# automl/learning_environments

Hardware: AMD Instinct MI355X
Metric: NES worker-evaluations/sec (full inner-loop train+eval) at pop=64 per GPU (higher is better)
Workload: dtype f32

## Files before the change

learning_environments_amd/csrc/dueling_se_inner_loop.hip:

```cpp
#include "lenv_gemm.cuh"
#include "lenv_ln.cuh"
#include "lenv_icm.cuh"
#include "lenv_wavechain_host.h"

namespace lenv {

constexpr int D_MAXL = 3;
constexpr int D_MAXW = 128;
constexpr int D_MAXH = 512;
constexpr int D_MAXB = 640;
constexpr int D_MAXI = 128;

struct DuelArena { int64_t a_online, a_target, a_m, a_v, a_grad, a_xs, a_xs2, a_act[D_MAXL], a_feat, a_v1, a_a1, a_t[6], a_dbuf[5], a_xh[D_MAXL], a_rstd, end; };
constexpr DuelArena duel_arena(int S, int H, int F, int L, int B, int T, int64_t P, bool ln = false)
{
    DuelArena a{};
    int64_t off = 0;
#define LENV_TAKE64(n) ([&]() { int64_t r_ = off; off += ((int64_t)(n) + 3) & ~(int64_t)3; return r_; }())
    a.a_online = LENV_TAKE64(P); a.a_target = LENV_TAKE64(P); a.a_m = LENV_TAKE64(P); a.a_v = LENV_TAKE64(P); a.a_grad = LENV_TAKE64(P);
    const int64_t rows = B > T ? B : T;
    const int W = H > F ? H : F;
    a.a_xs = LENV_TAKE64(rows * S); a.a_xs2 = LENV_TAKE64(rows * S);
    for (int l = 0; l < D_MAXL; ++l) a.a_act[l] = LENV_TAKE64(l < L ? (int64_t)B * H : 0);
    a.a_feat = LENV_TAKE64((int64_t)B * F); a.a_v1 = LENV_TAKE64((int64_t)B * F); a.a_a1 = LENV_TAKE64((int64_t)B * F);
// ... 218 lines not shown
            n_act = (int)rec[4]; learn_it = (int)rec[5]; n_test_ep = (int)rec[6]; train_steps = (int)rec[7]; test_steps = (int)rec[8];
            episodes_run = (int)rec[9];
            eps_g = __longlong_as_double(rec[11]); b1pow = __longlong_as_double(rec[12]); b2pow = __longlong_as_double(rec[13]);
            icm_pows[0] = __longlong_as_double(rec[14]); icm_pows[1] = __longlong_as_double(rec[15]);
        }
    }

    auto obs_of = [&](const double *st, float *obs) { real_env_obs(env_id, st, obs); };

    GemmQueue gq(cmds);
    constexpr int LNBUF = GemmShape<D_MAXI>::PS_FLOATS + GemmShape<D_MAXI>::QS_FLOATS;
    auto queue_forward = [&](const float *par, const float *X, int I, float *const *hid, float *featb, float *v1b, float *a1b, int slot,
                             float *const *xhs = nullptr, float *rstds = nullptr) {
        const float *in = X;
        int n_in = S;
        for (int l = 0; l < L; ++l) {
            if (ln && l >= 1) {
                gq.gemm(in, n_in, 1, par + po.oWf[l], n_in, 1, I, H, n_in, epi_bias(hid[l], H, 0, par + po.obf[l]));
                gq.run<D_MAXI>(Ps, Qs);
                ln_rows_forward<LNBUF>(Ps, hid[l], I, H, par + po.oLN, par + po.oLN + H, xhs ? xhs[l] : nullptr, rstds ? rstds + (int64_t)l * CFG_B : nullptr, act_id, prelu);
            } else gq.gemm(in, n_in, 1, par + po.oWf[l], n_in, 1, I, H, n_in, epi_bias_act(hid[l], H, par + po.obf[l], act_id, prelu));
            in = hid[l]; n_in = H;
        }
        if (plain) {
            gq.gemm(in, n_in, 1, par + po.oWf[L], n_in, 1, I, A, n_in, epi_bias(Advb + slot * RBH * A, A, 0, par + po.obf[L]));
            return;
        }
        gq.gemm(in, n_in, 1, par + po.oWf[L], n_in, 1, I, F, n_in, epi_bias(featb, F, 0, par + po.obf[L]));
        gq.gemm(featb, F, 1, par + po.oWv1, F, 1, I, F, F, epi_bias_act(v1b, F, par + po.obv1, act_id, prelu));
        gq.gemm(featb, F, 1, par + po.oWa1, F, 1, I, F, F, epi_bias_act(a1b, F, par + po.oba1, act_id, prelu));
        gq.gemm(v1b, F, 1, par + po.oWv2, F, 1, I, 1, F, epi_bias(Vb + slot * RBH, 1, 0, par + po.obv2));
        gq.gemm(a1b, F, 1, par + po.oWa2, F, 1, I, A, F, epi_bias(Advb + slot * RBH * A, A, 0, par + po.oba2));
    };
    auto finish_q = [&](int slot, int I, float *q_out, bool global_mean) {
        if (plain) {
            const float *src = Advb + slot * RBH * A;
            for (int e = tid; e < I * A; e += DNT) q_out[e] = src[e];
            __syncthreads();
            return;
        }
        const float *Vs = Vb + slot * RBH, *As = Advb + slot * RBH * A;
        if (global_mean) {
            if (tid == 0) {
                float sum = 0.0f;
                for (int e = 0; e < I * A; ++e) sum = sum + As[e];
                ctrl[8] = sum / (float)(I * A);
            }
            __syncthreads();
            const float mean = ctrl[8];
            for (int e = tid; e < I * A; e += DNT) q_out[e] = Vs[e / A] + (As[e] - mean);
        } else {
            for (int i = tid; i < I; i += DNT) {
                float sum = 0.0f;
                for (int aa = 0; aa < A; ++aa) sum = sum + As[i * A + aa];
                const float mean = sum / (float)A;
                for (int aa = 0; aa < A; ++aa) q_out[i * A + aa] = Vs[i] + (As[i * A + aa] - mean);
            }
        }
        __syncthreads();
    };
    auto forward = [&](const float *par, const float *X, int I, float *const *hid, float *featb, float *v1b, float *a1b,
                       float *q_out, bool global_mean) {
        queue_forward(par, X, I, hid, featb, v1b, a1b, 0);
        gq.run<D_MAXI>(Ps, Qs);
        finish_q(0, I, q_out, global_mean);
    };

    auto icm_step = [&]() {
        if constexpr (ICM) {
            IcmStep st{ gq, Ps, Qs, arena, a.a_icm, ctrl, 12, icm, icm_pows, cfg.icm_lr, cfg.icm_beta, cfg.icm_eta, cfg.adam_beta1, cfg.adam_beta2,
                        cfg.adam_eps, B, xs, S, xs2, S, false };
            const int Ai = icm.Ai;
            icm_train_and_reward<D_MAXI>(st, [&](int b, int i) { return Ai == 1 ? dAdv[b * A] : ((int)dAdv[b * A] == i ? 1.0f : 0.0f); },
                                         [&](int b, float r) { dAdv[b * A + 1] = dAdv[b * A + 1] + r; });
        }
    };

    float *hid_s[D_MAXL], *hid_t[D_MAXL];
    for (int l = 0; l < D_MAXL; ++l) { hid_s[l] = arena + AV(a_act[l]); hid_t[l] = arena + AV(a_t[l]); }
    float *xh_s[D_MAXL], *rstd_s = arena + AV(a_rstd);
    for (int l = 0; l < D_MAXL; ++l) xh_s[l] = arena + AV(a_xh[l]);
    float *feat_t = arena + AV(a_t[3]), *v1_t = arena + AV(a_t[4]), *a1_t = arena + AV(a_t[5]);

    auto test_phase = [&]() {
        if (tid < T) {
            double st[4];
            const int64_t row = (int64_t)n_test_ep + tid;
            if (tape) {
                if (row >= a.tapes.test_reset_stride) { status = -5; for (int i = 0; i < 4; ++i) st[i] = 0.0; }
                else for (int i = 0; i < 4; ++i) st[i] = a.tapes.test_reset[(chain * a.tapes.test_reset_stride + row) * 4 + i];
            } else {
                real_env_reset_draw(env_id, key, STREAM_TEST_RESET, row, st);
            }
            for (int i = 0; i < 4; ++i) dstate[tid * 4 + i] = st[i];
            ep_rew[tid] = 0.0f; alive[tid] = 1; tlen[tid] = 0;
        }
        if (tid == 0) ictrl[0] = 0;
        __syncthreads();
        float *xt = xs2;
        for (int t = 0; t < cfg.max_steps; t += k_rep) {
            if (tid < T) { float obs[8]; obs_of(dstate + tid * 4, obs); for (int i = 0; i < S; ++i) xt[tid * S + i] = obs[i]; }
            __syncthreads();
            forward(online, xt, T, hid_t, feat_t, v1_t, a1_t, qv, false);
            if (tid < T && alive[tid]) {
                int am = 0; float best = qv[tid * A];
                for (int aa = 1; aa < A; ++aa) { const float v = qv[tid * A + aa]; if (v > best) { best = v; am = aa; } }
                double st[4] = { dstate[tid * 4], dstate[tid * 4 + 1], dstate[tid * 4 + 2], dstate[tid * 4 + 3] };
                double rsum = 0.0;
                int nstep = 0;
                for (int r_ = 0; r_ < k_rep; ++r_) {
                    double rew; int dn;
                    real_env_step(env_id, st, am, rew, dn);
                    rsum = rsum + rew;
                    ++nstep;
                    if (tlen[tid] + nstep >= cfg.max_steps) dn = 1;
                    if (dn) { alive[tid] = 0; break; }
                }
                for (int i = 0; i < 4; ++i) dstate[tid * 4 + i] = st[i];
                ep_rew[tid] = ep_rew[tid] + (float)rsum;
                tlen[tid] = tlen[tid] + nstep;
                atomicAdd(const_cast<int *>(&ictrl[0]), nstep);
            }
            __syncthreads();
            int any = 0;
            for (int e = 0; e < T; ++e) any |= alive[e];
            if (!any) break;
        }
        if (tid < T) ret[tid] = (double)ep_rew[tid];
        n_test_ep += T;
        __syncthreads();
        test_steps += ictrl[0];
        __syncthreads();
    };

    const bool budgeted = cfg.step_budget > 0;
    const bool no_test_env = FIXED ? false : cfg.test_mode == 1;
// ... 12 lines not shown
                else for (int i = 0; i < 4; ++i) st0[i] = a.tapes.train_reset[(chain * a.tapes.train_reset_stride + episode) * 4 + i];
            } else {
                real_env_reset_draw(env_id, key, STREAM_TRAIN_RESET, episode, st0);
            }
            float obs[8];
            obs_of(st0, obs);
            for (int i = 0; i < S; ++i) state[i] = obs[i];
            if (reward_env) { for (int i = 0; i < 4; ++i) tstate[i] = st0[i]; ictrl[5] = 0; }
        }
        __syncthreads();
        int ep_len = 0, env_steps = 0;
        float tr_reward = 0.0f;
        for (int t = 0; t < cfg.max_steps; t += k_rep) {
            PT_MARK(9);
            const int size_after = train_steps + 1 < rb_cap ? train_steps + 1 : rb_cap;
            const int new_pos = train_steps % rb_cap;
            if (tid == 0) {
                double u;
                if (tape) { if (train_steps >= a.tapes.eps_uniform_stride) { status = -2; u = 1.0; } else u = a.tapes.eps_uniform[chain * a.tapes.eps_uniform_stride + train_steps]; }
                else u = u64_to_unit(rng_u64(key, STREAM_EPS, (uint64_t)train_steps));
                int explored = u < eps_g, action = -1;
                if (explored) {
                    if (tape) { if (n_act >= a.tapes.rand_action_stride) { status = -3; action = 0; } else action = a.tapes.rand_action[chain * a.tapes.rand_action_stride + n_act]; }
                    else action = (int)u64_to_below(rng_u64(key, STREAM_ACTION, (uint64_t)n_act), (uint32_t)A);
                }
                ictrl[1] = explored; ictrl[2] = action;
            }
            __syncthreads();
            const int explored = ictrl[1];
            if (explored) ++n_act;
            if (!explored) {
                for (int i = tid; i < S; i += DNT) xs2[i] = state[i];
                __syncthreads();
                forward(online, xs2, 1, hid_t, feat_t, v1_t, a1_t, qv, false);
                if (tid == 0) {
                    int am = 0; float best = qv[0];
                    for (int aa = 1; aa < A; ++aa) if (qv[aa] > best) { best = qv[aa]; am = aa; }
                    ictrl[2] = am;
                }
                __syncthreads();
            }
            const int action = ictrl[2];
            PT_MARK(0);
            if (reward_env) {
                auto rn_phi = [&](const float *obs, int slot) {
                    const float *rnp = seL > 1 ? arena + a.a_se_mid : rn_w;
                    const float *W0 = rnp, *b0 = rnp + Hse * Drn;
                    for (int j = tid; j < Hse; j += DNT) {
                        float z = 0.0f;
                        for (int k = 0; k < Drn; ++k) z = fma32(obs[k], W0[j * Drn + k], z);
                        rn_h[j] = act_fwd(se_act_id, cfg.se_prelu, z + b0[j]);
                    }
                    __syncthreads();
                    const float *hp = rn_h, *Wl = b0 + Hse;
                    float *hn = se_h2;
                    for (int l = 1; l < seL; ++l) {
                        const float *bl = Wl + Hse * Hse;
                        for (int j = tid; j < Hse; j += DNT) {
                            float z = 0.0f;
                            for (int k = 0; k < Hse; ++k) z = fma32(hp[k], Wl[j * Hse + k], z);
                            z = z + bl[j];
                            hn[j] = se_ln ? z : act_fwd(se_act_id, cfg.se_prelu, z);
                        }
                        __syncthreads();
                        if (se_ln) {
                            if (tid == 0) {
                                float sm = 0.0f, sv = 0.0f;
// ... 127 lines not shown
                a.out.trace_action[k] = action | (explored << 16);
                for (int i = 0; i < S; ++i) { a.out.trace_state[k * S + i] = newrow[i]; a.out.trace_next_state[k * S + i] = newrow[S + 1 + i]; }
                a.out.trace_reward_done[k * 2] = newrow[2 * S + 1]; a.out.trace_reward_done[k * 2 + 1] = newrow[2 * S + 2];
            }
            const float done_now = newrow[2 * S + 2];
            tr_reward = tr_reward + newrow[2 * S + 1];
            __syncthreads();
            if (tid < S) state[tid] = newrow[S + 1 + tid];
            ep_len += k_rep; ++train_steps;
            __syncthreads();
            PT_MARK(1);

            if (learning) {
                for (int b = tid; b < B; b += DNT) {
                    const int64_t n = (int64_t)learn_it * B + b;
                    int idx;
                    if (tape) {
                        if (n >= a.tapes.replay_idx_stride) { status = -4; idx = 0; } else idx = a.tapes.replay_idx[chain * a.tapes.replay_idx_stride + n];
                        if (idx < 0 || idx >= size_after) { status = -6; idx = 0; }
                    } else idx = (int)rng_replay_below(key, (uint64_t)n, (uint32_t)size_after);
                    const float *row = rb + (int64_t)idx * RS;
                    for (int i = 0; i < S; ++i) { xs[b * S + i] = row[i]; xs2[b * S + i] = row[S + 1 + i]; }
                    dAdv[b * A + 0] = row[S];
                    dAdv[b * A + 1] = row[2 * S + 1];
                    dq[b] = row[2 * S + 2];
                }
                __syncthreads();
                icm_step();
                PT_MARK(2);
                queue_forward(online, xs2, B, hid_t, feat_t, v1_t, a1_t, 1);
                queue_forward(target, xs2, B, hid_t, feat_t, v1_t, a1_t, 2);
                queue_forward(online, xs, B, hid_s, feat_s, v1_s, a1_s, 0, xh_s, rstd_s);
                gq.run<D_MAXI>(Ps, Qs);
                finish_q(1, B, qv + B * A, true);
                finish_q(2, B, qv + 2 * B * A, true);
                finish_q(0, B, qv, true);
                PT_MARK(3);
                for (int b = tid; b < B; b += DNT) {
                    const float g32 = (float)cfg.gamma, norm = (float)(2.0 / (double)B);
                    const int ab = (int)dAdv[b * A + 0];
                    const float r = dAdv[b * A + 1], d = dq[b];
                    int am = 0; float best = qv[(B + b) * A];
                    for (int aa = 1; aa < A; ++aa) { const float v = qv[(B + b) * A + aa]; if (v > best) { best = v; am = aa; } }
                    const float t1 = g32 * qv[(2 * B + b) * A + am];
                    const float t2 = 1.0f - d;
                    const float y = r + t1 * t2;
                    dq[b] = norm * (qv[b * A + ab] - y);
                    Vb[b] = (float)ab;
                }
                __syncthreads();
                if (tid == 0) {
                    float s_dq = 0.0f;
                    for (int b = 0; b < B; ++b) s_dq = s_dq + dq[b];
                    ctrl[9] = plain ? 0.0f : (-s_dq) / (float)(B * A);
                    b1pow *= cfg.adam_beta1; b2pow *= cfg.adam_beta2;
                    ctrl[10] = (float)(-(lr / (1.0 - b1pow)));
                    ctrl[11] = (float)__builtin_sqrt(1.0 - b2pow);
                }
                __syncthreads();
                {
                    const float mean_grad = ctrl[9];
                    for (int e = tid; e < B * A; e += DNT) {
                        const int b = e / A, aa = e - b * A;
                        const float g = aa == (int)Vb[b] ? dq[b] : 0.0f;
                        dAdv[e] = plain ? g : g + mean_grad;
                    }
                }
                __syncthreads();
                PT_MARK(4);
// ... 433 lines not shown
```

learning_environments_amd/csrc/dueling_wavechain.hip:

```cpp
#include "lenv_wavechain.cuh"
#ifndef WCT_NO_FUSED_OPT
#define WCT_FUSED_OPT
#endif
#include "lenv_wavechain_host.h"

namespace lenv {

using namespace wc;

struct WcShape { int env, S, A, Hse, T, q_act, se_act, kind; };
constexpr WcShape kWcShapes[] = {
    { -1, 2, 2, 1, 1, 0, 0, 1 },
    { LENV_ENV_ACROBOT, 6, 3, 128, 10, LENV_ACT_RELU, LENV_ACT_LEAKYRELU, 1 },
    { LENV_ENV_ACROBOT, 6, 3, 128, 10, LENV_ACT_RELU, LENV_ACT_LEAKYRELU, 0 },
};
constexpr int WC_B = 128, WC_H = 128;

namespace wcp {
constexpr int oW1t = 0, ob1 = 8 * W, oW2t = ob1 + W, ob2 = oW2t + IMG, oW3t = ob2 + W, ob3 = oW3t + IMG, oWv1t = ob3 + W, obv1 = oWv1t + IMG,
              oWa1t = obv1 + W, oba1 = oWa1t + IMG, oWh = oba1 + W, obh = oWh + 4 * W, PW = obh + 4;
static_assert(PW % 4 == 0, "float4 passes");
}

enum { D_H1 = 0, D_H2, D_FEAT, D_V1, D_A1, S_F1, S_DFEAT, S_DH2, S_DH1,
// ... 660 lines not shown
        sm_bias[i] = par[off + j];
    }
    for (int i = tid; i < 4 * W + 4; i += NT) sm_wh[i] = par[oWh + i];
    StageRegs sr;
    WSUB_DECL;
    stage_load_direct(par + oW2t, L, sr);
    stage_store_direct(bufA, L, sr);
    __syncthreads();
    WSUB_MARK(48);
    float r16[2][16], rf[2][64];
    f32x16 acc;
    auto xch = [&](int job) { return bufB + (quad * 2 + job) * 4096; };
#pragma unroll
    for (int j = 0; j < 2; ++j) {
        if (j < nj) {
            const float *X = pass == 0 ? xs2 : (j == 0 ? xs : xs2);
#pragma unroll
            for (int v = 0; v < 16; ++v) acc[v] = 0.0f;
            const lfloat *w1 = sm_w1t + L.h * W + 32 * jt + L.li;
#pragma unroll
            for (int t = 0; t < S / 2; ++t) acc = __builtin_amdgcn_mfma_f32_32x32x2f32(w1[2 * t * W], X[row * S + 2 * t + L.h], acc, 0, 0, 0);
#pragma unroll
            for (int g4 = 0; g4 < 4; ++g4) {
                const f32x4 bv = *(const lf4 *)(sm_bias + 32 * jt + 8 * g4 + 4 * L.h);
#pragma unroll
                for (int cc = 0; cc < 4; ++cc) r16[j][4 * g4 + cc] = act_fwd(ACT, prelu, acc[4 * g4 + cc] + bv[cc]);
            }
            if (pass == 1 && j == 0) piece_store(dump_of(D_H1, blk), jt, L.lane, r16[j]);
            tile16_to_operand(r16[j]);
            xch_put(xch(j), jt, L.lane, r16[j]);
        }
    }
    barrier_lds();
#pragma unroll
    for (int j = 0; j < 2; ++j) if (j < nj) xch_get(xch(j), L.lane, rf[j]);
    barrier_lds();
    WSUB_MARK(49);
#pragma unroll 1
    for (int l = 0; l < NL; ++l) {
#pragma unroll
        for (int j = 0; j < 2; ++j) {
            if (j < nj) {
#pragma unroll
                for (int v = 0; v < 16; ++v) acc[v] = 0.0f;
                chain_tile(bufA, jt, L, rf[j], acc);
                const lfloat *bb = sm_bias + (l + 1) * W + 32 * jt + 4 * L.h;
#pragma unroll
                for (int g4 = 0; g4 < 4; ++g4) {
                    const f32x4 bv = *(const lf4 *)(bb + 8 * g4);
#pragma unroll
                    for (int cc = 0; cc < 4; ++cc) {
                        const float z = acc[4 * g4 + cc] + bv[cc];
                        r16[j][4 * g4 + cc] = l == 1 ? z : act_fwd(ACT, prelu, z);
                    }
                }
                if (pass == 1 && j == 0) {
                    piece_store(dump_of(l == 0 ? D_H2 : (l == 1 ? D_FEAT : (l == 2 ? D_V1 : D_A1)), blk), jt, L.lane, r16[j]);
                    if (l >= 2 || PL) {
                        gfloat *rm = (gfloat *)dump_of(l == 2 ? R_V1 : R_A1, 0) + row * W + 32 * jt + 4 * L.h;
#pragma unroll
                        for (int g4 = 0; g4 < 4; ++g4) *(gf4 *)(rm + 8 * g4) = f32x4{r16[j][4 * g4], r16[j][4 * g4 + 1], r16[j][4 * g4 + 2], r16[j][4 * g4 + 3]};
                    }
                }
                tile16_to_operand(r16[j]);
            }
        }
        WSUB_MARK(50);
        if (!PL && l < 2) {
#pragma unroll
            for (int j = 0; j < 2; ++j) if (j < nj) xch_put(xch(j), jt, L.lane, r16[j]);
            barrier_lds();
#pragma unroll
            for (int j = 0; j < 2; ++j) if (j < nj) xch_get(xch(j), L.lane, rf[j]);
            stage_load_direct(par + (l == 0 ? oW3t : oWv1t), L, sr);
            stage_store_direct(bufA, L, sr);
            barrier_lds();
        } else if (!PL && l == 2) {
#pragma unroll
            for (int j = 0; j < 2; ++j) if (j < nj) xch_put(xch(j), jt, L.lane, r16[j]);
            barrier_lds();
            stage_load_direct(par + oWa1t, L, sr);
            stage_store_direct(bufA, L, sr);
            barrier_lds();
        } else {
            barrier_lds();
#pragma unroll
            for (int j = 0; j < 2; ++j) if (j < nj) xch_put(bufA + (quad * 2 + j) * 4096, jt, L.lane, r16[j]);
            barrier_lds();
            const int hd = wave & 1, tj = nj == 2 ? (wave >> 1) & 1 : 0, tq = nj == 2 ? wave >> 2 : wave >> 1;
            if ((nj == 2 || wave < 4) && !(PL && hd == 0)) {
                float rh[64];
                xch_get((hd == 0 ? bufB : bufA) + (tq * 2 + tj) * 4096, L.lane, rh);
                f32x16 hacc;
#pragma unroll
                for (int v = 0; v < 16; ++v) hacc[v] = 0.0f;
                const int col = hd == 0 ? 0 : 1 + (L.li < A ? L.li : A - 1);
                const lfloat *wh = sm_wh + L.h * 4 + col;
#pragma unroll
                for (int t = 0; t < 64; ++t) hacc = __builtin_amdgcn_mfma_f32_32x32x2f32(wh[2 * t * 4], rh[breg_of(t)], hacc, 0, 0, 0);
                if (L.h == 0) {
                    const int slot = pass == 0 ? 2 : tj, hrow = 32 * (2 * tg + tq) + L.li;
                    if (hd == 0) {
                        const float v = hacc[0] + sm_bh[0];
                        Vb_l[slot * RBH + hrow] = v;
                        gva[slot * B + hrow] = v;
                    } else {
#pragma unroll
                        for (int aa = 0; aa < A; ++aa) {
                            const float v = hacc[aa] + sm_bh[1 + aa];
                            Advb_l[slot * RBH * A + hrow * A + aa] = v;
                            gva[3 * B + (slot * B + hrow) * A + aa] = v;
                        }
                    }
                }
            }
        }
        WSUB_MARK(51);
    }
    __syncthreads();
    WSUB_MARK(52);
}

template <int SHAPE> static __device__ __noinline__ void wct_backward_chain(const WcCtx *ctx_)
{
    WCT_PROLOGUE;
    const int quad = wave >> 2, jt = wave & 3, blk = 2 * tg + quad, row = 32 * blk + L.li;
    constexpr bool PL = SP.kind == 0;
    constexpr int NQ = PL ? 1 : 4;
    float *xch = bufB + quad * 4096;
    for (int i = tid; i < 4 * W + 4; i += NT) sm_wh[i] = online[oWh + i];
    StageRegs sr;
    WSUB_DECL;
    stage_load_transposed(online + (PL ? oW2t : oWv1t), L, sr);
    __syncthreads();
    WSUB_MARK(53);
    float r16[16], f1[16], rf[64];
    f32x16 acc;
#pragma unroll 1
    for (int qi = 0; qi < NQ; ++qi) {
        const int q = PL ? 3 : qi, qu = PL ? 1 : qi;
        if (qu < 2) {
            f32x4 hv[4];
            piece_load(dump_of(PL ? D_H2 : (qu == 0 ? D_V1 : D_A1), blk), jt, L.lane, hv);
            const float dqi = dq_l[row];
            float da[A];
#pragma unroll
            for (int aa = 0; aa < A; ++aa) da[aa] = dAdv_l[row * A + aa];
#pragma unroll
            for (int g4 = 0; g4 < 4; ++g4) {
                const lfloat *whp = sm_wh + (32 * jt + 8 * g4 + 4 * L.h) * 4;
#pragma unroll
// ... 278 lines not shown
                  (float)(1.0 - cfg.tau), g, G, gva, dstate, ep_rew, alive, tlen, ret, reinterpret_cast<int *>(misc + 32), cfg.max_steps };
        *ctx = cx;
    }
    __syncthreads();

    const uint64_t key = a.rng_keys[chain];
    constexpr int env_id = SP.env;
    int status = 0;
    WPT_DECL;
    int train_steps = 0, n_act = 0, learn_it = 0, n_test_ep = 0, test_steps = 0, episodes_run = 0;
    double eps_g = cfg.eps_init, b1pow = 1.0, b2pow = 1.0;
    const int rb_cap = (int)a.rb_cap;
    TeamSync tsync{ team_bar, reinterpret_cast<unsigned *>(a.arena + a.a_bar) + 8, ictrl + 5, 0u, G, false, false };
    bool team_dead = false;
    auto team_barrier = [&]() {
        if (G == 1) return;
        wc::team_barrier<false>(tsync, tid);
        if (tsync.dead) { team_dead = true; status = -10; }
    };
    if (G > 1 && tid == 0) reinterpret_cast<unsigned *>(gva)[g] = __builtin_amdgcn_s_getreg((3 << 11) | 20) & 15u;
    team_barrier();
    if (G > 1) {
        bool same = true;
        const unsigned x0 = reinterpret_cast<unsigned *>(gva)[0];
        for (int m = 1; m < G; ++m) same = same && reinterpret_cast<unsigned *>(gva)[m] == x0;
        team_barrier();
        tsync.same_xcd = same;
    }
    if (team_dead) {
        if (a.out.status) atomicMin(&a.out.status[chain], -10);
        return;
    }

    auto finish_q = [&](int slot, int I, float *q_out, bool global_mean) {
        const float *Vs = Vb + slot * RBH, *As = Advb + slot * RBH * A;
        if constexpr (PL) {
            for (int e = tid; e < I * A; e += NT) q_out[e] = As[e];
        } else
        if (global_mean) {
            if (tid == 0) {
                float sum = 0.0f;
                for (int e = 0; e < I * A; ++e) sum = sum + As[e];
                ctrl[8] = sum / (float)(I * A);
            }
            __syncthreads();
            const float mean = ctrl[8];
            for (int e = tid; e < I * A; e += NT) q_out[e] = Vs[e / A] + (As[e] - mean);
        } else {
            for (int i = tid; i < I; i += NT) {
                float sum = 0.0f;
                for (int aa = 0; aa < A; ++aa) sum = sum + As[i * A + aa];
                const float mean = sum / (float)A;
                for (int aa = 0; aa < A; ++aa) q_out[i * A + aa] = Vs[i] + (As[i * A + aa] - mean);
            }
        }
        __syncthreads();
    };

    auto forward_thin = [&](const float *X, int I) {
        wc_forward_thin_layers<SHAPE>(ctx, X, I);
        finish_q(0, I, qv, false);
    };

    auto test_phase = [&]() {
        if constexpr (T <= 16) {
            __syncthreads();
            wc_test_steps<SHAPE>(ctx, (uint32_t)key, (uint32_t)(key >> 32), n_test_ep);
        } else {
            if (tid < T) {
                double st[4];
                real_env_reset_draw(env_id, key, STREAM_TEST_RESET, (int64_t)n_test_ep + tid, st);
                for (int i = 0; i < 4; ++i) dstate[tid * 4 + i] = st[i];
                ep_rew[tid] = 0.0f; alive[tid] = 1; tlen[tid] = 0;
            }
            if (tid == 0) ictrl[0] = 0;
            __syncthreads();
            float *xt = xscr;
            for (int t = 0; t < cfg.max_steps; ++t) {
                if (tid < T) { float obs[8]; real_env_obs(env_id, dstate + tid * 4, obs); for (int i = 0; i < S; ++i) xt[tid * S + i] = obs[i]; }
                __syncthreads();
                forward_thin(xt, T);
                if (tid < T && alive[tid]) {
                    int am = 0; float best = qv[tid * A];
                    for (int aa = 1; aa < A; ++aa) { const float v = qv[tid * A + aa]; if (v > best) { best = v; am = aa; } }
                    double st[4] = { dstate[tid * 4], dstate[tid * 4 + 1], dstate[tid * 4 + 2], dstate[tid * 4 + 3] };
                    double rew; int dn;
                    real_env_step(env_id, st, am, rew, dn);
                    for (int i = 0; i < 4; ++i) dstate[tid * 4 + i] = st[i];
                    ep_rew[tid] = ep_rew[tid] + (float)rew;
                    tlen[tid] = tlen[tid] + 1;
                    atomicAdd(reinterpret_cast<int *>(misc + 32), 1);
                    if (dn) alive[tid] = 0;
                }
                __syncthreads();
// ... 84 lines not shown
            ++ep_len; ++train_steps;
            __syncthreads();
            WPT_MARK(1);

            if (learning) {
                for (int b = tid; b < B; b += NT) {
                    const int64_t n = (int64_t)learn_it * B + b;
                    const int idx = (int)rng_replay_below(key, (uint64_t)n, (uint32_t)size_after);
                    const float *row = rb + (int64_t)idx * RS;
                    float rv[2 * S + 3];
#pragma unroll
                    for (int i = 0; i < 2 * S + 3; ++i) rv[i] = row[i];
#pragma unroll
                    for (int i = 0; i < S; ++i) { xs[b * S + i] = rv[i]; xs2[b * S + i] = rv[S + 1 + i]; }
                    dAdv[b * A + 0] = rv[S];
                    dAdv[b * A + 1] = rv[2 * S + 1];
                    dq[b] = rv[2 * S + 2];
                }
                __syncthreads();
                WPT_MARK(2);
#ifndef WC_DIAG_NO_FWD
                if (G == 2) {
#pragma unroll 1
                    for (int pass = 0; pass < 2; ++pass) wct_forward<SHAPE>(ctx, pass);
                    WBAR(60);
                    for (int e = tid; e < 3 * B; e += NT) Vb[(e / B) * RBH + (e % B)] = gva[e];
                    for (int e = tid; e < 3 * B * A; e += NT) Advb[(e / (B * A)) * RBH * A + (e % (B * A))] = gva[3 * B + e];
                    __syncthreads();
                } else {
#pragma unroll 1
                    for (int pass = 0; pass < 2; ++pass) wc_forward_big<SHAPE>(ctx, pass);
                }
#endif
                finish_q(1, B, qv + B * A, true);
                finish_q(2, B, qv + 2 * B * A, true);
                finish_q(0, B, qv, true);
                WPT_MARK(3);
                for (int b = tid; b < B; b += NT) {
                    const float g32 = (float)cfg.gamma, norm = (float)(2.0 / (double)B);
                    const int ab = (int)dAdv[b * A + 0];
                    const float rr = dAdv[b * A + 1], d = dq[b];
                    int am = 0; float best = qv[(B + b) * A];
                    for (int aa = 1; aa < A; ++aa) { const float v = qv[(B + b) * A + aa]; if (v > best) { best = v; am = aa; } }
                    const float t1 = g32 * qv[(2 * B + b) * A + am];
                    const float t2 = 1.0f - d;
                    const float y = rr + t1 * t2;
                    dq[b] = norm * (qv[b * A + ab] - y);
                    Vb[b] = (float)ab;
                }
                __syncthreads();
                if (tid == 0) {
                    float s_dq = 0.0f;
                    for (int b = 0; b < B; ++b) s_dq = s_dq + dq[b];
                    ctrl[9] = (-s_dq) / (float)(B * A);
                    b1pow *= cfg.adam_beta1; b2pow *= cfg.adam_beta2;
                    ctrl[10] = (float)(-(cfg.lr / (1.0 - b1pow)));
                    ctrl[11] = (float)__builtin_sqrt(1.0 - b2pow);
                }
                __syncthreads();
                {
                    const float mean_grad = ctrl[9];
                    for (int e = tid; e < B * A; e += NT) {
                        const int b = e / A, aa = e - b * A;
                        const float g = aa == (int)Vb[b] ? dq[b] : 0.0f;
                        dAdv[e] = PL ? g : g + mean_grad;
                    }
                }
                __syncthreads();
                WPT_MARK(4);
// ... 231 lines not shown
```

learning_environments_amd/csrc/lenv_gemm.cuh:

```cuda
#pragma once

#include "lenv_device.cuh"

namespace lenv {

#ifndef LENV_DNT
#define LENV_DNT 512
#endif
constexpr int DNT = LENV_DNT;
constexpr int DNW = DNT / 64;
constexpr int SKQ = 2048 / DNT;
constexpr int GT_I = 128, GT_J = 128, GT_RB = 64, GT_LD = 132;

enum { EPI_STORE = 0,
       EPI_BIAS_ACT = 1,
       EPI_BIAS = 2,
       EPI_ACT_BWD = 3,
       EPI_ACCUM = 4,
       EPI_BIAS_TANH = 5,
       EPI_BIAS_ADD = 6 };

enum { GEMM_GENERIC_P = 1, GEMM_GENERIC_OUT = 2 };

struct GemmEpi {
// ... 303 lines not shown
#pragma unroll
                    for (int v = 0; v < 16; ++v) acc[m][v] = fma32(prow[32 * bi[m] + 8 * (v >> 2) + (v & 3)], q, acc[m][v]);
                }
        }
#endif
    }
#ifdef LENV_DIAG_SKIP_EPI
    if (R > 0) return;
#endif
#pragma unroll
    for (int m = 0; m < NTW; ++m) {
        if (!has[m]) continue;
        if (ep.flags & GEMM_GENERIC_OUT) tile_epilogue<false, false>(acc[m], 32 * bi[m], 32 * bj[m], I, J, ep, lane);
        else if (32 * bi[m] + 32 <= I && 32 * bj[m] + 32 <= J) tile_epilogue<true, true>(acc[m], 32 * bi[m], 32 * bj[m], I, J, ep, lane);
        else tile_epilogue<true, false>(acc[m], 32 * bi[m], 32 * bj[m], I, J, ep, lane);
    }
}

__device__ __forceinline__ void wg_colsum(const float *d, int rows, int ld, int n, float *out)
{
    for (int k = (int)threadIdx.x; k < n; k += DNT) {
        float s = 0.0f;
        int b = 0;
        for (; b + 8 <= rows; b += 8) {
            float x[8];
#pragma unroll
            for (int u = 0; u < 8; ++u) x[u] = d[(int64_t)(b + u) * ld + k];
#pragma unroll
            for (int u = 0; u < 8; ++u) s = s + x[u];
        }
        for (; b < rows; ++b) s = s + d[(int64_t)b * ld + k];
        out[k] = s;
    }
}

template <int MAXI>
__device__ __noinline__ void gemm_run_queue(const GemmCmd *cmds_, int n_, float *Ps_, float *Qs_)
{
    typedef __attribute__((address_space(3))) const GemmCmd LCmd;
    const int tid = threadIdx.x, lane = tid & 63, wave = uni(tid >> 6);
    const int n = uni(n_);
    LCmd *cmds = (LCmd *)uni_ptr(cmds_);
    lfloat *Ps = (lfloat *)uni_ptr(Ps_), *Qs = (lfloat *)uni_ptr(Qs_);
    for (int k = 0; k < n; ++k) {
        LCmd &c = cmds[k];
        GemmOp op; GemmEpi ep;
        const int kind = uni(c.kind);
        op.P = uni_ptr(c.P); op.sPi = uni(c.sPi); op.sPr = uni(c.sPr); op.Q = uni_ptr(c.Q); op.sQj = uni(c.sQj); op.sQr = uni(c.sQr);
        op.I = uni(c.I); op.J = uni(c.J); op.R = uni(c.R);
        ep.kind = uni(c.ekind); ep.out = uni_ptr(c.out); ep.ldo = uni(c.ldo); ep.ocol = uni(c.ocol); ep.bias = uni_ptr(c.bias);
        ep.aux = uni_ptr(c.aux); ep.ldaux = uni(c.ldaux); ep.out2 = uni_ptr(c.out2); ep.ldo2 = uni(c.ldo2); ep.act = uni(c.act);
        ep.prelu = unif(c.prelu); ep.scale = unif(c.scale); ep.flags = uni(c.flags);
        if (kind == CMD_COLSUM) wg_colsum(op.P, op.I, op.sPi, op.J, ep.out);
        else if (op.I <= MAXI && op.J <= GT_J) gemm_body<MAXI>(op, ep, Ps, Qs, tid, lane, wave);
        else {
            const int I = op.I, J = op.J;
            const float *P0 = op.P, *Q0 = op.Q, *bias0 = ep.bias, *aux0 = ep.aux;
            float *out0 = ep.out, *out20 = ep.out2;
            for (int j0 = 0; j0 < J; j0 += GT_J)
                for (int i0 = 0; i0 < I; i0 += MAXI) {
                    if (i0 | j0) __syncthreads();
                    op.P = P0 + (int64_t)i0 * op.sPi; op.Q = Q0 + (int64_t)j0 * op.sQj;
                    op.I = I - i0 < MAXI ? I - i0 : MAXI; op.J = J - j0 < GT_J ? J - j0 : GT_J;
                    ep.out = out0 + (int64_t)i0 * ep.ldo + j0;
                    ep.bias = bias0 ? bias0 + j0 : nullptr;
                    ep.aux = aux0 ? aux0 + (int64_t)i0 * ep.ldaux + j0 : nullptr;
// ... 167 lines not shown
```

learning_environments_amd/csrc/lenv_wavechain.cuh:

```cuda
#pragma once

#include "lenv_gemm.cuh"

namespace lenv {
namespace wc {

constexpr int NT = 512, NW = 8;
constexpr int W = 128;
constexpr int IMG = W * W;
constexpr int BLK = 32 * W;

typedef __attribute__((address_space(1))) f32x4 gf4;
typedef __attribute__((address_space(3))) f32x4 lf4;

__device__ __forceinline__ void barrier_lds()
{
    asm volatile("s_waitcnt lgkmcnt(0)" ::: "memory");
    __builtin_amdgcn_s_barrier();
    asm volatile("" ::: "memory");
}

struct TeamSync {
    unsigned *bar, *launch_dead;
    volatile __attribute__((address_space(3))) int *lds_flag;
// ... 141 lines not shown
            *(lf4 *)(base + col) = f32x4{r[16 * jt + 4 * g], r[16 * jt + 4 * g + 1], r[16 * jt + 4 * g + 2], r[16 * jt + 4 * g + 3]};
        }
}

__device__ __forceinline__ void tile16_to_operand(float (&r)[16])
{
#pragma unroll
    for (int p = 0; p < 8; ++p) {
        auto s_ = __builtin_amdgcn_permlane32_swap(__float_as_uint(r[2 * p]), __float_as_uint(r[2 * p + 1]), false, false);
        r[2 * p] = __uint_as_float(s_[0]); r[2 * p + 1] = __uint_as_float(s_[1]);
    }
}
__device__ __forceinline__ void xch_put(float *xch_, int jt, int lane, const float (&r)[16])
{
    lfloat *x = (lfloat *)xch_ + (16 * jt) * 64 + lane;
#pragma unroll
    for (int v = 0; v < 16; ++v) x[v * 64] = r[v];
}
__device__ __forceinline__ void xch_get(const float *xch_, int lane, float (&r)[64])
{
    const lfloat *x = (const lfloat *)xch_ + lane;
#pragma unroll
    for (int v = 0; v < 64; ++v) r[v] = x[v * 64];
}
__device__ __forceinline__ void chain_tile(const float *img_, int jt, const Lane &L, const float (&b)[64], f32x16 &acc)
{
    const lfloat *img = (const lfloat *)img_;
    const lfloat *ab[4];
#pragma unroll
    for (int q = 0; q < 4; ++q) ab[q] = img + L.h * W + 32 * jt + L.colsw[q];
#pragma unroll
    for (int t = 0; t < 64; ++t) acc = __builtin_amdgcn_mfma_f32_32x32x2f32(ab[t & 3][2 * t * W], b[breg_of(t)], acc, 0, 0, 0);
}

struct StageRegs { f32x4 v[8]; };

__device__ __forceinline__ void stage_load_direct(const float *Wt, const Lane &L, StageRegs &s)
{
    const gf4 *src = (const gf4 *)Wt + L.tid;
#pragma unroll
    for (int u = 0; u < 8; ++u) s.v[u] = src[u * NT];
}
__device__ __forceinline__ void stage_store_direct(float *img_, const Lane &L, const StageRegs &s)
{
    lfloat *img = (lfloat *)img_;
#pragma unroll
    for (int u = 0; u < 8; ++u) {
        const int p = L.tid + u * NT, r = p >> 5, c = (p & 31) << 2;
        *(lf4 *)(img + r * W + (c ^ ((r & 7) << 2))) = s.v[u];
    }
}
__device__ __forceinline__ void stage_load_transposed(const float *Wt, const Lane &L, StageRegs &s)
{
#pragma unroll
    for (int u = 0; u < 8; ++u) {
        const int k = 16 * L.wave + (L.lane >> 2), c4 = 4 * u + (L.lane & 3);
        s.v[u] = *((const gf4 *)Wt + k * 32 + c4);
    }
}
__device__ __forceinline__ void stage_store_transposed(float *img_, const Lane &L, const StageRegs &s)
{
    lfloat *img = (lfloat *)img_;
#pragma unroll
    for (int u = 0; u < 8; ++u) {
        const int k = 16 * L.wave + (L.lane >> 2), c4 = 4 * u + (L.lane & 3);
#pragma unroll
// ... 296 lines not shown
```

Before: 2075.

## Overlap weight staging and exchange loads with MFMA chain; parallelize dueling mean reduction

The dueling forward chain is restructured: the next layer's weight image is loaded into registers before the current tile's MFMA chain, and the exchange-buffer reads for the second tile are interleaved into the MFMA loop via a new chain_tile_get. The head computation moves out of the layer loop. The three per-slot global-mean reductions, each previously a serial single-thread sum separated by barriers, are merged into one step where three waves each compute a slot's mean with a read-ahead unrolled sum, followed by one combined Q write. This aims to hide global and LDS latency behind MFMAs and cut barriers, at the cost of more register pressure and a changed summation code path.

After: 2072. No clear change (-0.1%).

```diff
diff --git a/learning_environments_amd/csrc/dueling_se_inner_loop.hip b/learning_environments_amd/csrc/dueling_se_inner_loop.hip
--- a/learning_environments_amd/csrc/dueling_se_inner_loop.hip
+++ b/learning_environments_amd/csrc/dueling_se_inner_loop.hip
@@ -274,7 +274,7 @@
         gq.gemm(v1b, F, 1, par + po.oWv2, F, 1, I, 1, F, epi_bias(Vb + slot * RBH, 1, 0, par + po.obv2));
         gq.gemm(a1b, F, 1, par + po.oWa2, F, 1, I, A, F, epi_bias(Advb + slot * RBH * A, A, 0, par + po.oba2));
     };
-    auto finish_q = [&](int slot, int I, float *q_out, bool global_mean) {
+    auto finish_q = [&](int slot, int I, float *q_out) {
         if (plain) {
             const float *src = Advb + slot * RBH * A;
             for (int e = tid; e < I * A; e += DNT) q_out[e] = src[e];
@@ -282,30 +282,36 @@
             return;
         }
         const float *Vs = Vb + slot * RBH, *As = Advb + slot * RBH * A;
-        if (global_mean) {
-            if (tid == 0) {
-                float sum = 0.0f;
-                for (int e = 0; e < I * A; ++e) sum = sum + As[e];
-                ctrl[8] = sum / (float)(I * A);
-            }
+        for (int i = tid; i < I; i += DNT) {
+            float sum = 0.0f;
+            for (int aa = 0; aa < A; ++aa) sum = sum + As[i * A + aa];
+            const float mean = sum / (float)A;
+            for (int aa = 0; aa < A; ++aa) q_out[i * A + aa] = Vs[i] + (As[i * A + aa] - mean);
+        }
+        __syncthreads();
+    };
+    auto finish_q_learn = [&]() {
+        if (plain) {
+            for (int e = tid; e < 3 * B * A; e += DNT) qv[e] = Advb[(e / (B * A)) * RBH * A + e % (B * A)];
             __syncthreads();
-            const float mean = ctrl[8];
-            for (int e = tid; e < I * A; e += DNT) q_out[e] = Vs[e / A] + (As[e] - mean);
-        } else {
-            for (int i = tid; i < I; i += DNT) {
-                float sum = 0.0f;
-                for (int aa = 0; aa < A; ++aa) sum = sum + As[i * A + aa];
-                const float mean = sum / (float)A;
-                for (int aa = 0; aa < A; ++aa) q_out[i * A + aa] = Vs[i] + (As[i * A + aa] - mean);
-            }
+            return;
+        }
+        if ((tid & 63) == 0 && tid < 3 * 64) {
+            const int slot = tid >> 6;
+            ctrl[26 + slot] = sum_ascending_ahead(Advb + slot * RBH * A, B * A) / (float)(B * A);
+        }
+        __syncthreads();
+        for (int e = tid; e < 3 * B * A; e += DNT) {
+            const int slot = e / (B * A), r = e - slot * (B * A);
+            qv[e] = Vb[slot * RBH + r / A] + (Advb[slot * RBH * A + r] - ctrl[26 + slot]);
         }
         __syncthreads();
     };
     auto forward = [&](const float *par, const float *X, int I, float *const *hid, float *featb, float *v1b, float *a1b,
-                       float *q_out, bool global_mean) {
+                       float *q_out) {
         queue_forward(par, X, I, hid, featb, v1b, a1b, 0);
         gq.run<D_MAXI>(Ps, Qs);
-        finish_q(0, I, q_out, global_mean);
+        finish_q(0, I, q_out);
     };
 
     auto icm_step = [&]() {
@@ -343,7 +349,7 @@
         for (int t = 0; t < cfg.max_steps; t += k_rep) {
             if (tid < T) { float obs[8]; obs_of(dstate + tid * 4, obs); for (int i = 0; i < S; ++i) xt[tid * S + i] = obs[i]; }
             __syncthreads();
-            forward(online, xt, T, hid_t, feat_t, v1_t, a1_t, qv, false);
+            forward(online, xt, T, hid_t, feat_t, v1_t, a1_t, qv);
             if (tid < T && alive[tid]) {
                 int am = 0; float best = qv[tid * A];
                 for (int aa = 1; aa < A; ++aa) { const float v = qv[tid * A + aa]; if (v > best) { best = v; am = aa; } }
@@ -422,7 +428,7 @@
             if (!explored) {
                 for (int i = tid; i < S; i += DNT) xs2[i] = state[i];
                 __syncthreads();
-                forward(online, xs2, 1, hid_t, feat_t, v1_t, a1_t, qv, false);
+                forward(online, xs2, 1, hid_t, feat_t, v1_t, a1_t, qv);
                 if (tid == 0) {
                     int am = 0; float best = qv[0];
                     for (int aa = 1; aa < A; ++aa) if (qv[aa] > best) { best = qv[aa]; am = aa; }
@@ -616,9 +622,7 @@
                 queue_forward(target, xs2, B, hid_t, feat_t, v1_t, a1_t, 2);
                 queue_forward(online, xs, B, hid_s, feat_s, v1_s, a1_s, 0, xh_s, rstd_s);
                 gq.run<D_MAXI>(Ps, Qs);
-                finish_q(1, B, qv + B * A, true);
-                finish_q(2, B, qv + 2 * B * A, true);
-                finish_q(0, B, qv, true);
+                finish_q_learn();
                 PT_MARK(3);
                 for (int b = tid; b < B; b += DNT) {
                     const float g32 = (float)cfg.gamma, norm = (float)(2.0 / (double)B);
diff --git a/learning_environments_amd/csrc/dueling_wavechain.hip b/learning_environments_amd/csrc/dueling_wavechain.hip
--- a/learning_environments_amd/csrc/dueling_wavechain.hip
+++ b/learning_environments_amd/csrc/dueling_wavechain.hip
@@ -716,91 +716,119 @@
         }
     }
     barrier_lds();
-#pragma unroll
-    for (int j = 0; j < 2; ++j) if (j < nj) xch_get(xch(j), L.lane, rf[j]);
+    xch_get(xch(0), L.lane, rf[0]);
     barrier_lds();
     WSUB_MARK(49);
-#pragma unroll 1
-    for (int l = 0; l < NL; ++l) {
-#pragma unroll
-        for (int j = 0; j < 2; ++j) {
-            if (j < nj) {
-#pragma unroll
-                for (int v = 0; v < 16; ++v) acc[v] = 0.0f;
-                chain_tile(bufA, jt, L, rf[j], acc);
-                const lfloat *bb = sm_bias + (l + 1) * W + 32 * jt + 4 * L.h;
-#pragma unroll
-                for (int g4 = 0; g4 < 4; ++g4) {
-                    const f32x4 bv = *(const lf4 *)(bb + 8 * g4);
-#pragma unroll
-                    for (int cc = 0; cc < 4; ++cc) {
-                        const float z = acc[4 * g4 + cc] + bv[cc];
-                        r16[j][4 * g4 + cc] = l == 1 ? z : act_fwd(ACT, prelu, z);
-                    }
+    auto epilogue = [&](int l, float (&r)[16], bool keep) {
+        const lfloat *bb = sm_bias + (l + 1) * W + 32 * jt + 4 * L.h;
+#pragma unroll
+        for (int g4 = 0; g4 < 4; ++g4) {
+            const f32x4 bv = *(const lf4 *)(bb + 8 * g4);
+#pragma unroll
+            for (int cc = 0; cc < 4; ++cc) {
+                const float z = acc[4 * g4 + cc] + bv[cc];
+                r[4 * g4 + cc] = l == 1 ? z : act_fwd(ACT, prelu, z);
+            }
+        }
+        if (keep) {
+            piece_store(dump_of(l == 0 ? D_H2 : (l == 1 ? D_FEAT : (l == 2 ? D_V1 : D_A1)), blk), jt, L.lane, r);
+            if (l >= 2 || PL) {
+                gfloat *rm = (gfloat *)dump_of(l == 2 ? R_V1 : R_A1, 0) + (32 * blk + L.li) * W + 32 * jt + 4 * L.h;
+#pragma unroll
+                for (int g4 = 0; g4 < 4; ++g4) *(gf4 *)(rm + 8 * g4) = f32x4{r[4 * g4], r[4 * g4 + 1], r[4 * g4 + 2], r[4 * g4 + 3]};
+            }
+        }
+        tile16_to_operand(r);
+    };
+    auto next_image = [&](int l) { return par + (l == 0 ? oW3t : (l == 1 ? oWv1t : oWa1t)); };
+    if (nj == 1) {
+#pragma unroll
+        for (int l = 0; l < NL; ++l) {
+            L.refresh();
+            const bool more = !PL && l < 3;
+            StageRegs nx;
+            if (more) stage_load_direct(next_image(l), L, nx);
+            __builtin_amdgcn_sched_barrier(0);
+#pragma unroll
+            for (int v = 0; v < 16; ++v) acc[v] = 0.0f;
+            chain_tile(bufA, jt, L, rf[0], acc);
+            epilogue(l, r16[0], false);
+            WSUB_MARK(50);
+            if (more) {
+                xch_put(xch(0), jt, L.lane, r16[0]);
+                barrier_lds();
+                if (l < 2) xch_get(xch(0), L.lane, rf[0]);
+                stage_store_direct(bufA, L, nx);
+                barrier_lds();
+                WSUB_MARK(51);
+            }
+        }
+    } else {
+#pragma unroll
+        for (int l = 0; l < NL; ++l) {
+            L.refresh();
+            const bool more = !PL && l < 3;
+#pragma unroll
+            for (int v = 0; v < 16; ++v) acc[v] = 0.0f;
+            if (l < 3) chain_tile_get(bufA, jt, L, rf[0], acc, xch(1), rf[1]);
+            else chain_tile(bufA, jt, L, rf[0], acc);
+            epilogue(l, r16[0], true);
+            WSUB_MARK(50);
+            if (more) {
+                xch_put(xch(0), jt, L.lane, r16[0]);
+                barrier_lds();
+            }
+            WSUB_MARK(51);
+            StageRegs nx;
+            if (more) stage_load_direct(next_image(l), L, nx);
+            __builtin_amdgcn_sched_barrier(0);
+#pragma unroll
+            for (int v = 0; v < 16; ++v) acc[v] = 0.0f;
+            if (more && l < 2) chain_tile_get(bufA, jt, L, rf[1], acc, xch(0), rf[0]);
+            else chain_tile(bufA, jt, L, rf[1], acc);
+            epilogue(l, r16[1], false);
+            WSUB_MARK(50);
+            if (more) {
+                xch_put(xch(1), jt, L.lane, r16[1]);
+                barrier_lds();
+                stage_store_direct(bufA, L, nx);
+                barrier_lds();
+                WSUB_MARK(51);
+            }
+        }
+    }
+    barrier_lds();
+#pragma unroll
+    for (int j = 0; j < 2; ++j) if (j < nj) xch_put(bufA + (quad * 2 + j) * 4096, jt, L.lane, r16[j]);
+    barrier_lds();
+    const int hd = wave & 1, tj = nj == 2 ? (wave >> 1) & 1 : 0, tq = nj == 2 ? wave >> 2 : wave >> 1;
+    if ((nj == 2 || wave < 4) && !(PL && hd == 0)) {
+        float rh[64];
+        xch_get((hd == 0 ? bufB : bufA) + (tq * 2 + tj) * 4096, L.lane, rh);
+        f32x16 hacc;
+#pragma unroll
+        for (int v = 0; v < 16; ++v) hacc[v] = 0.0f;
+        const int col = hd == 0 ? 0 : 1 + (L.li < A ? L.li : A - 1);
+        const lfloat *wh = sm_wh + L.h * 4 + col;
+#pragma unroll
+        for (int t = 0; t < 64; ++t) hacc = __builtin_amdgcn_mfma_f32_32x32x2f32(wh[2 * t * 4], rh[breg_of(t)], hacc, 0, 0, 0);
+        if (L.h == 0) {
+            const int slot = pass == 0 ? 2 : tj, hrow = 32 * (2 * tg + tq) + L.li;
+            if (hd == 0) {
+                const float v = hacc[0] + sm_bh[0];
+                Vb_l[slot * RBH + hrow] = v;
+                gva[slot * B + hrow] = v;
+            } else {
+#pragma unroll
+                for (int aa = 0; aa < A; ++aa) {
+                    const float v = hacc[aa] + sm_bh[1 + aa];
+                    Advb_l[slot * RBH * A + hrow * A + aa] = v;
+                    gva[3 * B + (slot * B + hrow) * A + aa] = v;
                 }
-                if (pass == 1 && j == 0) {
-                    piece_store(dump_of(l == 0 ? D_H2 : (l == 1 ? D_FEAT : (l == 2 ? D_V1 : D_A1)), blk), jt, L.lane, r16[j]);
-                    if (l >= 2 || PL) {
-                        gfloat *rm = (gfloat *)dump_of(l == 2 ? R_V1 : R_A1, 0) + row * W + 32 * jt + 4 * L.h;
-#pragma unroll
-                        for (int g4 = 0; g4 < 4; ++g4) *(gf4 *)(rm + 8 * g4) = f32x4{r16[j][4 * g4], r16[j][4 * g4 + 1], r16[j][4 * g4 + 2], r16[j][4 * g4 + 3]};
-                    }
-                }
-                tile16_to_operand(r16[j]);
-            }
-        }
-        WSUB_MARK(50);
-        if (!PL && l < 2) {
-#pragma unroll
-            for (int j = 0; j < 2; ++j) if (j < nj) xch_put(xch(j), jt, L.lane, r16[j]);
-            barrier_lds();
-#pragma unroll
-            for (int j = 0; j < 2; ++j) if (j < nj) xch_get(xch(j), L.lane, rf[j]);
-            stage_load_direct(par + (l == 0 ? oW3t : oWv1t), L, sr);
-            stage_store_direct(bufA, L, sr);
-            barrier_lds();
-        } else if (!PL && l == 2) {
-#pragma unroll
-            for (int j = 0; j < 2; ++j) if (j < nj) xch_put(xch(j), jt, L.lane, r16[j]);
-            barrier_lds();
-            stage_load_direct(par + oWa1t, L, sr);
-            stage_store_direct(bufA, L, sr);
-            barrier_lds();
-        } else {
-            barrier_lds();
-#pragma unroll
-            for (int j = 0; j < 2; ++j) if (j < nj) xch_put(bufA + (quad * 2 + j) * 4096, jt, L.lane, r16[j]);
-            barrier_lds();
-            const int hd = wave & 1, tj = nj == 2 ? (wave >> 1) & 1 : 0, tq = nj == 2 ? wave >> 2 : wave >> 1;
-            if ((nj == 2 || wave < 4) && !(PL && hd == 0)) {
-                float rh[64];
-                xch_get((hd == 0 ? bufB : bufA) + (tq * 2 + tj) * 4096, L.lane, rh);
-                f32x16 hacc;
-#pragma unroll
-                for (int v = 0; v < 16; ++v) hacc[v] = 0.0f;
-                const int col = hd == 0 ? 0 : 1 + (L.li < A ? L.li : A - 1);
-                const lfloat *wh = sm_wh + L.h * 4 + col;
-#pragma unroll
-                for (int t = 0; t < 64; ++t) hacc = __builtin_amdgcn_mfma_f32_32x32x2f32(wh[2 * t * 4], rh[breg_of(t)], hacc, 0, 0, 0);
-                if (L.h == 0) {
-                    const int slot = pass == 0 ? 2 : tj, hrow = 32 * (2 * tg + tq) + L.li;
-                    if (hd == 0) {
-                        const float v = hacc[0] + sm_bh[0];
-                        Vb_l[slot * RBH + hrow] = v;
-                        gva[slot * B + hrow] = v;
-                    } else {
-#pragma unroll
-                        for (int aa = 0; aa < A; ++aa) {
-                            const float v = hacc[aa] + sm_bh[1 + aa];
-                            Advb_l[slot * RBH * A + hrow * A + aa] = v;
-                            gva[3 * B + (slot * B + hrow) * A + aa] = v;
-                        }
-                    }
-                }
-            }
-        }
-        WSUB_MARK(51);
-    }
+            }
+        }
+    }
+    WSUB_MARK(51);
     __syncthreads();
     WSUB_MARK(52);
 }
@@ -1145,20 +1173,10 @@
         return;
     }
 
-    auto finish_q = [&](int slot, int I, float *q_out, bool global_mean) {
+    auto finish_q = [&](int slot, int I, float *q_out) {
         const float *Vs = Vb + slot * RBH, *As = Advb + slot * RBH * A;
         if constexpr (PL) {
             for (int e = tid; e < I * A; e += NT) q_out[e] = As[e];
-        } else
-        if (global_mean) {
-            if (tid == 0) {
-                float sum = 0.0f;
-                for (int e = 0; e < I * A; ++e) sum = sum + As[e];
-                ctrl[8] = sum / (float)(I * A);
-            }
-            __syncthreads();
-            const float mean = ctrl[8];
-            for (int e = tid; e < I * A; e += NT) q_out[e] = Vs[e / A] + (As[e] - mean);
         } else {
             for (int i = tid; i < I; i += NT) {
                 float sum = 0.0f;
@@ -1169,10 +1187,26 @@
         }
         __syncthreads();
     };
+    auto finish_q_learn = [&]() {
+        if constexpr (PL) {
+            for (int e = tid; e < 3 * B * A; e += NT) qv[e] = Advb[(e / (B * A)) * RBH * A + e % (B * A)];
+        } else {
+            if ((tid & 63) == 0 && tid < 3 * 64) {
+                const int slot = tid >> 6;
+                ctrl[26 + slot] = sum_ascending_ahead(Advb + slot * RBH * A, B * A) / (float)(B * A);
+            }
+            __syncthreads();
+            for (int e = tid; e < 3 * B * A; e += NT) {
+                const int slot = e / (B * A), r = e - slot * (B * A);
+                qv[e] = Vb[slot * RBH + r / A] + (Advb[slot * RBH * A + r] - ctrl[26 + slot]);
+            }
+        }
+        __syncthreads();
+    };
 
     auto forward_thin = [&](const float *X, int I) {
         wc_forward_thin_layers<SHAPE>(ctx, X, I);
-        finish_q(0, I, qv, false);
+        finish_q(0, I, qv);
     };
 
     auto test_phase = [&]() {
@@ -1323,9 +1357,7 @@
                     for (int pass = 0; pass < 2; ++pass) wc_forward_big<SHAPE>(ctx, pass);
                 }
 #endif
-                finish_q(1, B, qv + B * A, true);
-                finish_q(2, B, qv + 2 * B * A, true);
-                finish_q(0, B, qv, true);
+                finish_q_learn();
                 WPT_MARK(3);
                 for (int b = tid; b < B; b += NT) {
                     const float g32 = (float)cfg.gamma, norm = (float)(2.0 / (double)B);
diff --git a/learning_environments_amd/csrc/lenv_gemm.cuh b/learning_environments_amd/csrc/lenv_gemm.cuh
--- a/learning_environments_amd/csrc/lenv_gemm.cuh
+++ b/learning_environments_amd/csrc/lenv_gemm.cuh
@@ -359,6 +359,31 @@
         for (; b < rows; ++b) s = s + d[(int64_t)b * ld + k];
         out[k] = s;
     }
+}
+
+__device__ __forceinline__ float sum_ascending_ahead(const float *p, int n)
+{
+    constexpr int U = 32;
+    float s = 0.0f;
+    int e = 0;
+    if (n >= U) {
+        float cur[U];
+#pragma unroll
+        for (int u = 0; u < U; ++u) cur[u] = p[u];
+        for (e = U; e + U <= n; e += U) {
+            float nxt[U];
+#pragma unroll
+            for (int u = 0; u < U; ++u) nxt[u] = p[e + u];
+#pragma unroll
+            for (int u = 0; u < U; ++u) s = s + cur[u];
+#pragma unroll
+            for (int u = 0; u < U; ++u) cur[u] = nxt[u];
+        }
+#pragma unroll
+        for (int u = 0; u < U; ++u) s = s + cur[u];
+    }
+    for (; e < n; ++e) s = s + p[e];
+    return s;
 }
 
 template <int MAXI>
diff --git a/learning_environments_amd/csrc/lenv_wavechain.cuh b/learning_environments_amd/csrc/lenv_wavechain.cuh
--- a/learning_environments_amd/csrc/lenv_wavechain.cuh
+++ b/learning_environments_amd/csrc/lenv_wavechain.cuh
@@ -197,6 +197,19 @@
 #pragma unroll
     for (int t = 0; t < 64; ++t) acc = __builtin_amdgcn_mfma_f32_32x32x2f32(ab[t & 3][2 * t * W], b[breg_of(t)], acc, 0, 0, 0);
 }
+__device__ __forceinline__ void chain_tile_get(const float *img_, int jt, const Lane &L, const float (&b)[64], f32x16 &acc, const float *xch_, float (&g)[64])
+{
+    const lfloat *img = (const lfloat *)img_;
+    const lfloat *x = (const lfloat *)xch_ + L.lane;
+    const lfloat *ab[4];
+#pragma unroll
+    for (int q = 0; q < 4; ++q) ab[q] = img + L.h * W + 32 * jt + L.colsw[q];
+#pragma unroll
+    for (int t = 0; t < 64; ++t) {
+        acc = __builtin_amdgcn_mfma_f32_32x32x2f32(ab[t & 3][2 * t * W], b[breg_of(t)], acc, 0, 0, 0);
+        g[t] = x[t * 64];
+    }
+}
 
 struct StageRegs { f32x4 v[8]; };
 
```
